# vision-agh/apse_uav

Measured on AMD Instinct MI355X. Metric: 4K UAV frames/sec (whole node), higher is better.
Workload: dtype f32

## Files before the change

### apse_uav_amd/_lib.py

```python
import ctypes as C
import os

import numpy as np

_HERE = os.path.dirname(os.path.abspath(__file__))
_TREE_LIB = os.path.join(_HERE, "libapse_hip.so")
LIB_PATH = os.environ.get("APSE_HIP_LIB") or _TREE_LIB
TOOL_ENTRIES = ("apse_winograd_pack_filter", "apse_winograd_conv2d", "apse_lane_stats", "apse_rpn_select", "apse_box_inference",
                "apse_c4_rpn_select", "apse_rpn_select_train", "apse_rpn_train_proposals_workspace_bytes", "apse_rpn_train_proposals",
                "apse_set_rpn_head", "apse_preprocess_frames_yuv", "apse_yuv_to_bgr", "apse_yuv_matrix_host", "apse_resize_normalize_yuv")

APSE_OK = 0


class ApseError(RuntimeError):
    pass


class Config(C.Structure):
    _fields_ = [
        ("struct_size", C.c_int), ("device", C.c_int), ("max_batch", C.c_int),
        ("frame_h", C.c_int), ("frame_w", C.c_int), ("image_h", C.c_int), ("image_w", C.c_int),
        ("blocks", C.c_int * 4), ("num_classes", C.c_int),
        ("score_thresh", C.c_float), ("box_nms", C.c_float), ("rpn_nms", C.c_float), ("mask_thresh", C.c_float),
        ("rpn_pre_topk", C.c_int), ("rpn_post_topk", C.c_int), ("dets_per_image", C.c_int),
        ("pixel_mean", C.c_float * 3), ("assoc_roi", C.c_int), ("embed_dim", C.c_int), ("assoc_scale", C.c_float),
        ("compute_dtype", C.c_int), ("storage16", C.c_int),
    ]


class ConfigArch(Config):
# ... 48 lines not shown
    "apse_set_detections": ([vp, vp, vp, vp, vp, i, vp], i),
    "apse_mask_tail": ([vp, i, vp], i),
    "apse_embed": ([vp, i, vp], i),
    "apse_forward": ([vp, i, vp], i),
    "apse_results_describe": ([vp, C.POINTER(ResultsLayout)], i),
    "apse_read_results": ([vp, vp, sz, vp], i),
    "apse_read_results_begin": ([vp, vp, sz, vp], i),
    "apse_read_results_end": ([vp, vp], i),
    "apse_lane_stats": ([vp, C.POINTER(C.c_longlong * 4)], i),
    "apse_copy_mask_window": ([vp, i, i, i, i, i, vp, vp], i),
    "apse_copy_mask_windows": ([vp, i, vp, vp, vp, vp, vp], i),
    "apse_host_copy": ([vp, vp, sz, i], i),
    "apse_feature_shape": ([vp, C.c_char_p, C.POINTER(C.c_int * 3)], i),
    "apse_export_feature": ([vp, C.c_char_p, vp, i, vp], i),
    "apse_debug_tensor": ([vp, C.c_char_p, vp, sz, C.POINTER(sz), vp], i),
    "apse_flops": ([vp, i, C.c_double, C.c_double], C.c_double),
    "apse_profile": ([vp, i], i),
    "apse_profile_read": ([vp, C.POINTER(C.c_double * 42), i], i),
    "apse_conv_packed_elems": ([C.POINTER(ConvDesc)], sz),
    "apse_conv_pack_weight": ([C.POINTER(ConvDesc), vp, i, vp, vp], i),
    "apse_conv2d": ([C.POINTER(ConvDesc), vp, vp, vp, vp, vp, vp, sz, vp], i),
    "apse_winograd_pack_filter": ([vp, i, i, vp], i),
    "apse_winograd_conv2d": ([C.POINTER(ConvDesc), vp, vp, vp, vp, vp], i),
    "apse_maxpool3x3s2": ([vp, vp, i, i, i, i, vp], i),
    "apse_maxpool3x3s2_typed": ([vp, vp, i, i, i, i, i, vp], i),
    "apse_roi_align": ([C.POINTER(vp), C.POINTER(i), C.POINTER(i), vp, i, i, i, vp, vp], i),
    "apse_roi_align_typed": ([C.POINTER(vp), C.POINTER(i), C.POINTER(i), vp, i, i, i, i, vp, vp], i),
    "apse_roi_pool": ([vp, i, i, vp, vp, i, i, f, vp, vp], i),
    "apse_roi_features": ([vp, i, vp, vp, i, i, vp, vp], i),
    "apse_nms_rank": ([vp, vp, vp, i, i, i, i, f, i, vp, vp, vp, vp, vp], i),
    "apse_rpn_select": ([C.POINTER(vp), C.POINTER(i), C.POINTER(i), i, i, i, i, i, i, f, i, vp, vp, vp, vp, vp, vp, vp, vp, vp], i),
    "apse_box_inference": ([vp, i, i, vp, vp, i, i, i, i, f, f, i, i] + [vp] * 16, i),
    "apse_c4_rpn_select": ([vp, i, i, i, i, i, i, i, f, vp, vp, vp, vp, vp, vp, vp, vp], i),
    "apse_mask_centroid_dense": ([vp, i, i, C.POINTER(C.c_int * 3), vp], i),
    "apse_mask_closest_dense": ([vp, i, i, f, f, C.POINTER(C.c_int * 2), vp], i),
    "apse_l2_normalize": ([vp, vp, i, i, vp], i),
    "apse_sqdist": ([vp, vp, i, i, i, vp, vp], i),
    "apse_undistort_gamma": ([vp, vp, i, i, i, C.POINTER(C.c_double), C.POINTER(C.c_double), i, vp, i, i, vp], i),
    "apse_lab_tables_host": ([vp, vp, C.c_size_t], C.c_size_t),
    "apse_replay_create": ([i, i, f, i], vp),
    "apse_replay_destroy": ([vp], None),
    "apse_replay_step": ([vp, i, i, vp, vp, vp, C.c_char_p, i, vp], i),
    "apse_replay_packed": ([vp, vp, C.c_longlong, i, i, i, vp, C.c_longlong], C.c_longlong),
    "apse_replay_max_id": ([vp], i),
    "apse_replay_next_id": ([vp], i),
    "apse_render_workspace_bytes": ([i, i, i], sz),
# ... 116 lines not shown
```

### apse_uav_amd/csrc/apse_common.h

```cpp
#pragma once
#include <hip/hip_runtime.h>
#include <stdint.h>

#define APSE_OK 0
#define APSE_E_INVALID (-1)
#define APSE_E_HIP (-2)
#define APSE_E_NOMEM (-3)
#define APSE_E_STATE (-4)
#define APSE_E_MISSING (-5)
#define APSE_MAX_FRAME_W 49152
#define APSE_MAX_FRAME_H 32768
#define APSE_MAX_CLASSES 80
#define APSE_LDS_BYTES 163840

int apse_fail_global(int code, const char* msg);

typedef __attribute__((ext_vector_type(16))) float f32x16;
typedef __attribute__((ext_vector_type(4))) float f32x4;

struct ConvParams {
    const float* x;
    const float* w;
    const uint16_t* w16;
    const float* bias;
// ... 2 lines not shown
    float* ws;
    int* tile_cnt;
    const int* m_count;
    int m_per_item;
    int m_hint;
    int B, H, W, cin_log2;
    int OH, OW, Cout;
    int KH, KW, stride, pad;
    int KWCp;
    int M;
    int relu;
    int res_mode;
    int out_mode;
    int y_ld, y_coff;
    int cdec;
    int splitk;
    int steps_total;
    const void* next_w;
    unsigned next_w_bytes;
    int prec;
    int x_st, res_st, y_st;
    int no_stream;
    const float* wu;
};

int apse_launch_conv(const ConvParams& p, int cfg, hipStream_t s, hipEvent_t ev0 = nullptr, hipEvent_t ev1 = nullptr);
int apse_conv_pick_cfg(int M, int Cout, int steps, int* splitk);
#define APSE_CFG_STREAM 9
#define APSE_CFG_BNECK 10
#define APSE_CFG_GLDS 11
#define APSE_CFG_STEMPOOL 12
#define APSE_CFG_SKINNY 13
#define APSE_NCFG 14
bool apse_conv1x1_stream_ok(const ConvParams& p);
int apse_launch_conv1x1_stream(const ConvParams& p, hipStream_t s, hipEvent_t ev0 = nullptr, hipEvent_t ev1 = nullptr);
bool apse_conv_glds16_ok(const ConvParams& p);
bool apse_conv_glds16_small(const ConvParams& p);
bool apse_conv_skinny_ok(const ConvParams& p);
int apse_launch_conv_skinny(const ConvParams& p, hipStream_t s, hipEvent_t ev0 = nullptr, hipEvent_t ev1 = nullptr);
int apse_launch_conv_glds16(const ConvParams& p, hipStream_t s, hipEvent_t ev0 = nullptr, hipEvent_t ev1 = nullptr);
int apse_conv_effective_cfg(const ConvParams& p, int cfg);
bool apse_conv_winograd_ok(const ConvParams& p, int max_items);
int apse_conv_winograd_blocks(const ConvParams& p);
int apse_launch_conv_winograd(const ConvParams& p, hipStream_t s, hipEvent_t ev0 = nullptr, hipEvent_t ev1 = nullptr);
typedef __bf16 bf16x8 __attribute__((ext_vector_type(8)));

#ifdef __HIPCC__
typedef _Float16 f16x4_t __attribute__((ext_vector_type(4)));
typedef __bf16 bf16x4_t __attribute__((ext_vector_type(4)));
__device__ __forceinline__ int apse_xcd_remap(int wg, int nwg) {
    const int q = nwg >> 3, r = nwg & 7, xcd = wg & 7, idx = wg >> 3;
    return (xcd < r ? xcd * (q + 1) : r * (q + 1) + (xcd - r) * q) + idx;
}
__device__ __forceinline__ f32x4 apse_ld4(const void* base, size_t idx, int st) {
    if (st == 0) return *reinterpret_cast<const f32x4*>(reinterpret_cast<const float*>(base) + idx);
    f32x4 r;
    if (st == 1) {
        const uint2 raw = *reinterpret_cast<const uint2*>(reinterpret_cast<const uint16_t*>(base) + idx);
        r[0] = __uint_as_float(raw.x << 16); r[1] = __uint_as_float(raw.x & 0xffff0000u);
        r[2] = __uint_as_float(raw.y << 16); r[3] = __uint_as_float(raw.y & 0xffff0000u);
    } else {
        const f16x4_t h = *reinterpret_cast<const f16x4_t*>(reinterpret_cast<const uint16_t*>(base) + idx);
        r[0] = (float)h[0]; r[1] = (float)h[1]; r[2] = (float)h[2]; r[3] = (float)h[3];
    }
    return r;
}
// ... 88 lines not shown
```

### apse_uav_amd/csrc/conv_igemm.hip

```cpp
#include "apse_common.h"
#include <type_traits>

typedef _Float16 f16x8 __attribute__((ext_vector_type(8)));
__device__ __forceinline__ f32x16 apse_mfma16(bf16x8 a, bf16x8 b, f32x16 c) { return __builtin_amdgcn_mfma_f32_32x32x16_bf16(a, b, c, 0, 0, 0); }
__device__ __forceinline__ f32x16 apse_mfma16(f16x8 a, f16x8 b, f32x16 c) { return __builtin_amdgcn_mfma_f32_32x32x16_f16(a, b, c, 0, 0, 0); }

template <int WM, int WN, int TM, int TN, int KS, int XT, int WK, int PR = 0>
__global__ __launch_bounds__(64 * WM * WN * WK) void conv_igemm_f32(const ConvParams p) {
    static_assert(PR == 0 || XT == 0, "16-bit operands use the descriptor path only");
    constexpr bool DESC = XT != 1;
    constexpr int EPS = PR ? 64 : 32;
    constexpr int ESH = PR ? 1 : 2;
    constexpr int EPSLOT = 16 >> ESH;
    constexpr int NT = 64 * WM * WN * WK;
    constexpr int BM = WM * TM * 32;
    constexpr int BN = WN * TN * 32;
    constexpr int SR = NT / 8;
    constexpr int AP = BM / SR;
    constexpr int BP = BN / SR;
    static_assert(AP >= 1 && BP >= 1 && KS % WK == 0 && (DESC || WK == 1), "unsupported shape");
    constexpr int LDC = BN + 4;
    constexpr bool DP = DESC && (TM * TN <= 2 || (PR != 0 && WM * WN == 8 && APSE_DP16));
    constexpr int NSET = DP ? 2 : 1;
    constexpr int STORE_AT = 4 * KS - 2;
// ... 584 lines not shown
        if (p.out_mode == 0) {
            if (p.res_mode == 1) {
                val += ld1((size_t)m * p.Cout + n);
            } else if (p.res_mode == 2) {
                const int b = m / ohw;
                const int rem = m - b * ohw;
                const int oy = rem / p.OW, ox = rem - oy * p.OW;
                const int hw2 = (p.OH >> 1) * (p.OW >> 1);
                val += ld1(((size_t)b * hw2 + (oy >> 1) * (p.OW >> 1) + (ox >> 1)) * p.Cout + n);
            }
            dst = (size_t)m * p.y_ld + p.y_coff + n;
        } else {
            const int b = m / ohw;
            const int rem = m - b * ohw;
            const int oy = rem / p.OW, ox = rem - oy * p.OW;
            const int dy = g >> 1, dx = g & 1;
            dst = (((size_t)b * 2 * p.OH + 2 * oy + dy) * (2 * p.OW) + 2 * ox + dx) * p.cdec + co;
        }
        if (p.relu) val = apse_relu(val);
        apse_st1(p.y, dst, val, p.y_st);
    }
}

template <int WM, int WN, int TM, int TN, int KS, int XT, int WK = 1, int PR = 0>
static int launch_cfg_x(const ConvParams& p, hipStream_t s, hipEvent_t ev0, hipEvent_t ev1) {
    constexpr int BM = WM * TM * 32, BN = WN * TN * 32;
    const int tiles = ((p.M + BM - 1) / BM) * ((p.Cout + BN - 1) / BN);
    const size_t lds_stage = (size_t)2 * KS * (BM + BN) * 32 * sizeof(float), lds_c = (size_t)WK * BM * (BN + 4) * sizeof(float) + 16;
    const size_t lds = lds_stage > lds_c ? lds_stage : lds_c;
    static bool attr_done = false;
    if (!attr_done) {
        hipFuncSetAttribute(reinterpret_cast<const void*>(&conv_igemm_f32<WM, WN, TM, TN, KS, XT, WK, PR>),
                            hipFuncAttributeMaxDynamicSharedMemorySize, (int)lds);
        attr_done = true;
    }
    int grid_x = tiles;
    if (p.m_count) {
        int want = 1024;
        if (p.m_hint > 0) {
            want = 2 * ((p.m_hint + BM - 1) / BM) * ((p.Cout + BN - 1) / BN);
            if (want < 64) want = 64;
            if (want > 1024) want = 1024;
        }
        if (grid_x > want) grid_x = want;
    }
    if (ev0) hipEventRecord(ev0, s);
// ... 138 lines not shown
```

### apse_uav_amd/csrc/conv_winograd.hip

```cpp
#include "apse_common.h"

namespace {
constexpr int WTR = 16, WTC = 4;
constexpr int WT = WTR * WTC;
constexpr int WN = 64;
constexpr int KC = 8;
constexpr int NTHR = 512;
constexpr int G_U = 1, G_ROWS = 2, G_V = 3;
constexpr int SLICE_F = 16 * WT * KC;
constexpr size_t WINO_LDS = (size_t)2 * 2 * SLICE_F * sizeof(float);
static_assert(WN == WT, "V and U slices share one size");
static_assert((size_t)16 * WT * 32 * sizeof(float) <= WINO_LDS, "epilogue chunk must fit the staging LDS");
}

__global__ __launch_bounds__(NTHR) void conv_winograd_f32(const ConvParams p) {
    extern __shared__ __attribute__((aligned(16))) char smem[];
    float* Vs = reinterpret_cast<float*>(smem);
    float* Us = Vs + 2 * SLICE_F;
    float* Cs = reinterpret_cast<float*>(smem);

    const int tid = threadIdx.x;
    const int lane = tid & 63, wave = __builtin_amdgcn_readfirstlane(tid >> 6);
    const int fr = lane & 31, fh = lane >> 5;

    const int tiles_y = (p.OH + 2 * WTR - 1) / (2 * WTR), tiles_x = (p.OW + 2 * WTC - 1) / (2 * WTC);
    const int nblk = p.Cout / WN;
    const int nwg = p.B * tiles_y * tiles_x * nblk;
    const int bid = apse_xcd_remap(blockIdx.x, nwg);
    const int nb = bid % nblk;
    int rest = bid / nblk;
    const int bx = rest % tiles_x; rest /= tiles_x;
    const int by = rest % tiles_y;
    const int b = rest / tiles_y;
    const int oy0 = by * 2 * WTR, ox0 = bx * 2 * WTC, n0 = nb * WN;
    const int C = 1 << p.cin_log2;
    const int nsteps = C / KC;

    const int cg = tid & 1, t = (tid >> 1) & (WT - 1), ti = wave >> 1;
    const int ra = ti == 0 ? 0 : (ti == 2 ? 2 : 1);
    const int rb = ti == 0 ? 2 : (ti == 1 ? 2 : (ti == 2 ? 1 : 3));
    const float sgn = ti == 1 ? 1.f : -1.f;
    const int iy_a = oy0 + 2 * (t / WTC) - 1 + ra, iy_b = oy0 + 2 * (t / WTC) - 1 + rb;
    const int ix0 = ox0 + 2 * (t % WTC) - 1;
    const __amdgpu_buffer_rsrc_t xrsrc =
        __builtin_amdgcn_make_buffer_rsrc(const_cast<float*>(p.x), 0, (int)((((unsigned)(p.B * p.H * p.W)) << p.cin_log2) * 4u), 0x00020000);
    const __amdgpu_buffer_rsrc_t xnone = __builtin_amdgcn_make_buffer_rsrc(const_cast<float*>(p.x), 0, 0, 0x00020000);
    unsigned xoff[2][4];
#pragma unroll
    for (int r = 0; r < 2; ++r) {
        const int iy = r ? iy_b : iy_a;
#pragma unroll
        for (int c = 0; c < 4; ++c) {
            const int ix = ix0 + c;
            const bool in = (unsigned)iy < (unsigned)p.H && (unsigned)ix < (unsigned)p.W;
            xoff[r][c] = in ? ((((unsigned)((b * p.H + iy) * p.W + ix)) << p.cin_log2) + (unsigned)(cg * 4)) * 4u : 0x80000000u;
        }
    }
    const __amdgpu_buffer_rsrc_t ursrc =
        __builtin_amdgcn_make_buffer_rsrc(const_cast<float*>(p.wu), 0, (int)((((unsigned)(16 * p.Cout)) << p.cin_log2) * 4u), 0x00020000);
    const unsigned ustep = (unsigned)(16 * p.Cout * KC * 4);
    unsigned uoff[4], ulds[4];
#pragma unroll
    for (int k = 0; k < 4; ++k) {
        const int q = tid + NTHR * k;
        const int xi = q >> 7, co = (q >> 1) & 63, h = q & 1;
        uoff[k] = (unsigned)(((xi * p.Cout + n0 + co) * KC + h * 4) * 4);
        ulds[k] = (unsigned)((xi * WN + co) * KC + ((h ^ ((co >> 3) & 1)) * 4));
    }
    const int vlds = (4 * ti * WT + t) * KC + (cg ^ ((t >> 3) & 1)) * 4;

    f32x4 xr[2][4], ur[4];
    auto fetch_u = [&](int s) {
        const unsigned kb = (unsigned)s * ustep;
#pragma unroll
        for (int k = 0; k < 4; ++k) ur[k] = __builtin_bit_cast(f32x4, __builtin_amdgcn_raw_buffer_load_b128(ursrc, (int)(uoff[k] + kb), 0, 0));
    };
    auto fetch_x = [&](int s) {
        const unsigned kb = (unsigned)(s * KC * 4);
        const __amdgpu_buffer_rsrc_t rs = s < nsteps ? xrsrc : xnone;
#pragma unroll
        for (int r = 0; r < 2; ++r)
#pragma unroll
            for (int c = 0; c < 4; ++c)
                xr[r][c] = __builtin_bit_cast(f32x4, __builtin_amdgcn_raw_buffer_load_b128(rs, (int)(xoff[r][c] + kb), 0, 0));
    };
    auto write_u = [&](int buf) {
#pragma unroll
        for (int k = 0; k < 4; ++k) *reinterpret_cast<f32x4*>(Us + buf * SLICE_F + ulds[k]) = ur[k];
    };
    auto xform_rows = [&]() {
#pragma unroll
        for (int c = 0; c < 4; ++c)
#pragma unroll
            for (int e = 0; e < 4; ++e) xr[0][c][e] = __builtin_fmaf(xr[1][c][e], sgn, xr[0][c][e]);
    };
    auto write_v = [&](int buf) {
        const f32x4 v[4] = {xr[0][0] - xr[0][2], xr[0][1] + xr[0][2], xr[0][2] - xr[0][1], xr[0][1] - xr[0][3]};
#pragma unroll
        for (int j = 0; j < 4; ++j) *reinterpret_cast<f32x4*>(Vs + buf * SLICE_F + vlds + j * WT * KC) = v[j];
    };

// ... 58 lines not shown
    typedef unsigned u32x4_t __attribute__((ext_vector_type(4)));
#pragma unroll
    for (int j = 0; j < 2; ++j) {
#pragma unroll
        for (int a = 0; a < 2; ++a)
#pragma unroll
            for (int i = 0; i < 2; ++i)
#pragma unroll
                for (int v = 0; v < 16; ++v) {
                    const int row = 32 * i + (v & 3) + 8 * (v >> 2) + 4 * fh;
                    Cs[((2 * wave + a) * WT + row) * 32 + fr] = acc[a][i][j][v];
                }
        __syncthreads();
        f32x4 m[16];
#pragma unroll
        for (int k = 0; k < 16; ++k) m[k] = *reinterpret_cast<const f32x4*>(Cs + (k * WT + et) * 32 + eg * 4);
        f32x4 s0[4], s1[4];
#pragma unroll
        for (int c = 0; c < 4; ++c) {
            s0[c] = m[c] + m[4 + c] + m[8 + c];
            s1[c] = m[4 + c] - m[8 + c] - m[12 + c];
        }
        const int co = n0 + 32 * j + 4 * eg;
        const f32x4 bias4 = p.bias ? *reinterpret_cast<const f32x4*>(p.bias + co) : f32x4{0.f, 0.f, 0.f, 0.f};
        f32x4 y[2][2] = {{s0[0] + s0[1] + s0[2], s0[1] - s0[2] - s0[3]}, {s1[0] + s1[1] + s1[2], s1[1] - s1[2] - s1[3]}};
#pragma unroll
        for (int dy = 0; dy < 2; ++dy)
#pragma unroll
            for (int dx = 0; dx < 2; ++dx) {
                f32x4 val = y[dy][dx] + bias4;
                if (p.relu) {
#pragma unroll
                    for (int k = 0; k < 4; ++k) val[k] = apse_relu(val[k]);
                }
                if (oy + dy < p.OH && ox + dx < p.OW)
                    APSE_NT_STORE(val, reinterpret_cast<f32x4*>(p.y + ((size_t)(b * p.OH + oy + dy) * p.OW + ox + dx) * p.y_ld + p.y_coff + co));
            }
        __syncthreads();
    }
}

bool apse_conv_winograd_ok(const ConvParams& p, int max_items) {
    return p.prec == 0 && p.x_st == 0 && p.y_st == 0 && p.KH == 3 && p.KW == 3 && p.stride == 1 && p.pad == 1 && p.out_mode == 0 &&
           p.res_mode == 0 && p.splitk == 1 && p.Cout % WN == 0 && p.cin_log2 >= 3 && p.OH == p.H && p.OW == p.W &&
           (p.y_ld & 3) == 0 && (p.y_coff & 3) == 0 && ((((size_t)max_items * p.H * p.W) << p.cin_log2) * 4 < 0x7fff0000ull);
}

int apse_conv_winograd_blocks(const ConvParams& p) {
    return ((p.OH + 2 * WTR - 1) / (2 * WTR)) * ((p.OW + 2 * WTC - 1) / (2 * WTC)) * (p.Cout / WN);
}

int apse_launch_conv_winograd(const ConvParams& p, hipStream_t s, hipEvent_t ev0, hipEvent_t ev1) {
    if (!p.wu || !apse_conv_winograd_ok(p, p.B) || p.m_count) return APSE_E_INVALID;
    static bool attr_done = false;
    if (!attr_done) {
        hipFuncSetAttribute(reinterpret_cast<const void*>(&conv_winograd_f32), hipFuncAttributeMaxDynamicSharedMemorySize, (int)WINO_LDS);
        attr_done = true;
    }
    const int tiles_y = (p.OH + 2 * WTR - 1) / (2 * WTR), tiles_x = (p.OW + 2 * WTC - 1) / (2 * WTC);
    const int grid = p.B * tiles_y * tiles_x * (p.Cout / WN);
    if (ev0) hipEventRecord(ev0, s);
    hipLaunchKernelGGL(conv_winograd_f32, dim3(grid), dim3(NTHR), WINO_LDS, s, p);
    if (ev1) hipEventRecord(ev1, s);
    return hipGetLastError() == hipSuccess ? APSE_OK : APSE_E_HIP;
}
```

### apse_uav_amd/csrc/ops.hip

```cpp
#include "detector_ctx.h"

#include <math.h>
#include <string.h>

#include <map>
#include <mutex>
#include <vector>

namespace {
struct DevBuf {
    void* p = nullptr;
    ~DevBuf() { if (p) hipFree(p); }
    bool alloc(size_t bytes, bool zero = false) {
        if (hipMalloc(&p, bytes ? bytes : 16) != hipSuccess) { p = nullptr; return false; }
        if (zero) hipMemset(p, 0, bytes ? bytes : 16);
        return true;
    }
    template <typename T> T* as() const { return reinterpret_cast<T*>(p); }
};
}

extern "C" {

size_t apse_conv_packed_elems(const apse_conv_desc* d) {
// ... 61 lines not shown
}

int apse_winograd_pack_filter(const float* w, int Cout, int Cin, float* packed) {
    if (!w || !packed || Cout < 1 || Cin < 8 || pow2_at_least(Cin) != Cin) return APSE_E_INVALID;
    const std::vector<float> u = winograd_filters(w, Cout, Cin, Cin);
    memcpy(packed, u.data(), u.size() * sizeof(float));
    return APSE_OK;
}

int apse_winograd_conv2d(const apse_conv_desc* d, const float* x, const float* wu, const float* bias, float* y, void* stream) {
    if (!d || !x || !wu || !y || d->B < 1 || d->H < 1 || d->W < 1 || d->Cin < 8 || pow2_at_least(d->Cin) != d->Cin) return APSE_E_INVALID;
    ConvParams p;
    memset(&p, 0, sizeof p);
    p.x = x; p.wu = wu; p.bias = bias; p.y = y;
    p.B = d->B; p.H = d->H; p.W = d->W; p.cin_log2 = apse_ilog2(d->Cin);
    p.KH = d->KH; p.KW = d->KW; p.stride = d->stride; p.pad = d->pad;
    p.OH = d->H; p.OW = d->W; p.Cout = d->Cout; p.relu = d->relu;
    p.M = p.B * p.OH * p.OW; p.m_per_item = p.OH * p.OW;
    p.y_ld = d->Cout; p.splitk = 1;
    p.res_mode = d->res_mode; p.prec = d->prec; p.x_st = d->x_st; p.y_st = d->y_st;
    return apse_launch_conv_winograd(p, (hipStream_t)stream);
}

int apse_maxpool3x3s2(const float* x, float* y, int B, int H, int W, int C, void* stream) {
    return apse_k_maxpool3x3s2(x, y, B, H, W, C, 0, (hipStream_t)stream);
}

int apse_maxpool3x3s2_typed(const void* x, void* y, int B, int H, int W, int C, int storage, void* stream) {
    if (!x || !y || B < 1 || H < 1 || W < 1 || C < 4 || (C & 3) || storage < 0 || storage > 2) return APSE_E_INVALID;
    return apse_k_maxpool3x3s2(x, y, B, H, W, C, storage, (hipStream_t)stream);
}

static int roi_align_stateless(const void* const* feats, const int* hs, const int* ws, const float* rois, int n, int per_img,
                               int out_size, int st, void* out, void* stream) {
    if (!feats || !hs || !ws || !rois || !out || n < 0 || out_size < 1 || st < 0 || st > 2) return APSE_E_INVALID;
    FpnMaps F;
    static const float sc[4] = {0.25f, 0.125f, 0.0625f, 0.03125f};
    for (int l = 0; l < 4; ++l) { F.p[l] = feats[l]; F.H[l] = hs[l]; F.W[l] = ws[l]; F.scale[l] = sc[l]; }
    F.st = st;
    static int* total_dev = nullptr;
    if (!total_dev) hipMalloc(reinterpret_cast<void**>(&total_dev), sizeof(int));
    hipMemcpyAsync(total_dev, &n, sizeof(int), hipMemcpyHostToDevice, (hipStream_t)stream);
    hipStreamSynchronize((hipStream_t)stream);
    std::vector<int> img(n);
    for (int i = 0; i < n; ++i) img[i] = per_img > 0 ? i / per_img : 0;
    int* img_dev = nullptr;
// ... 343 lines not shown
```

### apse_uav_amd/csrc/plan.hip

```cpp
#include "detector_ctx.h"

#include <math.h>
#include <stdio.h>
#include <string.h>

#define APSE_WINO_MIN_BLOCKS 128
#define APSE_EXPECTED_DETS 8

void pack_oihw(const float* w, int Cout, int Cin, int KH, int KW, int cin_p, const float* scale, float* out, int KWCp) {
    for (int o = 0; o < Cout; ++o) {
        const float sc = scale ? scale[o] : 1.0f;
        for (int r = 0; r < KH; ++r)
            for (int s = 0; s < KW; ++s)
                for (int ci = 0; ci < Cin; ++ci)
                    out[((size_t)o * KH + r) * KWCp + s * cin_p + ci] = w[(((size_t)o * Cin + ci) * KH + r) * KW + s] * sc;
    }
}

static const HostW* getw(apse_ctx* c, const std::string& n) {
    auto it = c->hw.find(n);
    return it == c->hw.end() ? nullptr : &it->second;
}

static Tens make_t(apse_ctx* c, const std::string& name, int items, int H, int W, int C, int st = 0) {
    Tens t;
    t.H = H; t.W = W; t.C = C; t.st = st;
    const size_t elems = (size_t)items * H * W * C;
    t.p = dalloc<float>(c, st ? (elems + 1) / 2 : elems);
    c->t[name] = t;
// ... 11 lines not shown
    const Tens* res = nullptr; int res_mode = 0;
    int y_ld = 0;
    int count_kind = 0;
    float* out_ptr = nullptr;
    const Tens* out_view = nullptr;
};

static uint16_t round16(float v, int dtype) {
    if (dtype == 2) {
        const _Float16 hval = (_Float16)v;
        uint16_t r;
        memcpy(&r, &hval, 2);
        return r;
    }
    uint32_t b;
    memcpy(&b, &v, 4);
    if ((b & 0x7fffffffu) > 0x7f800000u) return (uint16_t)((b >> 16) | 0x40);
    return (uint16_t)((b + 0x7fffu + ((b >> 16) & 1u)) >> 16);
}
static int storage_type(const apse_ctx* c) { return (c->cfg.compute_dtype >= 1 && c->cfg.storage16) ? c->cfg.compute_dtype : 0; }

static bool winograd_layer(const std::string& n) {
    return n == "backbone.fpn_output2" || n == "backbone.fpn_output3" || n == "rpn_t2" || n == "rpn_t3";
}
std::vector<float> winograd_filters(const float* oihw, int Cout, int Cin, int cin_p) {
    static const double G[4][3] = {{1, 0, 0}, {0.5, 0.5, 0.5}, {0.5, -0.5, 0.5}, {0, 0, 1}};
    std::vector<float> u((size_t)16 * Cout * cin_p, 0.f);
    for (int o = 0; o < Cout; ++o)
        for (int ci = 0; ci < Cin; ++ci) {
            const float* g = oihw + ((size_t)o * Cin + ci) * 9;
            double t[4][3];
            for (int i = 0; i < 4; ++i)
                for (int s = 0; s < 3; ++s) t[i][s] = G[i][0] * g[s] + G[i][1] * g[3 + s] + G[i][2] * g[6 + s];
            for (int i = 0; i < 4; ++i)
                for (int j = 0; j < 4; ++j) {
                    const double v = t[i][0] * G[j][0] + t[i][1] * G[j][1] + t[i][2] * G[j][2];
                    u[(((size_t)(ci / 8) * 16 + 4 * i + j) * Cout + o) * 8 + (ci & 7)] = (float)v;
                }
        }
    return u;
}

static int add_conv(apse_ctx* c, std::vector<Step>& plan, const ConvSpec& sp, const Tens& in, Tens* out) {
    const std::string& out_name = sp.out_name.empty() ? sp.name : sp.out_name;
    std::vector<float> rows;
    std::vector<float> bias;
// ... 118 lines not shown
    Tens o;
    if (sp.out_view) { o = *sp.out_view; o.H = oh; o.W = ow; o.C = out_c; c->t[out_name] = o; }
    else if (sp.out_ptr) { o.p = sp.out_ptr; o.H = oh; o.W = ow; o.C = out_c; }
    else o = make_t(c, out_name, c->cfg.max_batch * sp.items, oh, ow, out_c, out_st);
    p.y_st = o.st;
    if (!o.p) return fail(c, APSE_E_NOMEM, "activation alloc failed at " + sp.name);
    p.y = o.p; p.y_ld = out_c; p.y_coff = 0;
    cs.flops_per_item = sp.s2d ? 2.0 * p.OH * p.OW * (double)Cout * 7 * 7 * 3
                               : 2.0 * p.OH * p.OW * (double)Cout * KH * KW * Cin;
    const int Mfull = c->cfg.max_batch * sp.items * p.OH * p.OW;
    int sk = 1;
    cs.cfg = apse_conv_pick_cfg(Mfull, Cout, p.steps_total, &sk);
    if (sp.count_kind == 2) {
        const int kd = c->cfg.dets_per_image < APSE_EXPECTED_DETS ? c->cfg.dets_per_image : APSE_EXPECTED_DETS;
        const int rows = kd * c->cfg.max_batch * p.OH * p.OW;
        sk = 1;
        cs.cfg = apse_conv_pick_cfg(rows < Mfull ? rows : Mfull, Cout, p.steps_total, &sk);
    }
    p.splitk = sk;
    if (sk > 1) {
        const size_t need = (size_t)sk * Mfull * Cout;
        if (need > c->ws_floats) c->ws_floats = need;
    }
    if (c->f32_winograd && winograd_layer(sp.name) && sp.count_kind == 0 && apse_conv_winograd_ok(p, c->cfg.max_batch * sp.items) &&
        apse_conv_winograd_blocks(p) >= APSE_WINO_MIN_BLOCKS) {
        p.wu = dupload(c, winograd_filters(rows.data(), Cout, Cin, cin_p));
        if (!p.wu) return fail(c, APSE_E_NOMEM, "weight upload failed at " + sp.name);
    }
    if (out) *out = o;
    plan.push_back(st);
    return APSE_OK;
}

static void layout_results(apse_ctx* c) {
    apse_results_layout& L = c->lay;
    memset(&L, 0, sizeof(L));
    const int B = c->cfg.max_batch, kd = c->cfg.dets_per_image, n = B * kd, E = c->cfg.embed_dim;
    L.n_max = n; L.dets_per_image = kd; L.embed_dim = E; L.max_batch = B;
    size_t o = 0;
    auto take = [&](size_t bytes) { size_t r = o; o += (bytes + 15) / 16 * 16; return r; };
    L.total = take(4);
    L.offset = take(4 * (B + 1));
    L.prop_count = take(4 * B);
    L.img = take(4 * n); L.cls = take(4 * n); L.roi = take(4 * n); L.score = take(4 * n);
    L.box_resized = take(16 * n); L.box = take(16 * n); L.valid = take(4 * n); L.rect = take(16 * n);
    L.mass = take(4 * n); L.centroid = take(8 * n);
    L.closest = take((size_t)8 * n * kd);
    L.embedding = take((size_t)4 * n * E);
    L.bytes = o;
}
// ... 480 lines not shown
```

### apse_uav_amd/winograd.py

```python
import numpy as np

BT = np.array([[1, 0, -1, 0], [0, 1, 1, 0], [0, -1, 1, 0], [0, 1, 0, -1]], dtype=np.float64)
G = np.array([[1, 0, 0], [0.5, 0.5, 0.5], [0.5, -0.5, 0.5], [0, 0, 1]], dtype=np.float64)
AT = np.array([[1, 1, 1, 0], [0, 1, -1, -1]], dtype=np.float64)


def filter_transform(w):
    w = np.asarray(w, dtype=np.float64)
    u = np.einsum("ir,ocrs,js->ijoc", G, w, G)
    return u.reshape(16, w.shape[0], w.shape[1]).astype(np.float32)


def _input_transform(d):
    d0, d1, d2, d3 = d[..., 0, :, :], d[..., 1, :, :], d[..., 2, :, :], d[..., 3, :, :]
    rows = [d0 - d2, d1 + d2, d2 - d1, d1 - d3]
    v = []
    for x in rows:
        x0, x1, x2, x3 = x[..., 0, :], x[..., 1, :], x[..., 2, :], x[..., 3, :]
        v += [x0 - x2, x1 + x2, x2 - x1, x1 - x3]
    return np.stack(v, axis=-2)


def _output_transform(m):
    q = [m[..., k, :] for k in range(16)]
    s0 = [q[0 + j] + q[4 + j] + q[8 + j] for j in range(4)]
    s1 = [q[4 + j] - q[8 + j] - q[12 + j] for j in range(4)]
    y00 = s0[0] + s0[1] + s0[2]
    y01 = s0[1] - s0[2] - s0[3]
    y10 = s1[0] + s1[1] + s1[2]
    y11 = s1[1] - s1[2] - s1[3]
    return np.stack([np.stack([y00, y01], -2), np.stack([y10, y11], -2)], -3)


def emulate(x_hwc, w_oihw, bias, relu):
    x = np.asarray(x_hwc, dtype=np.float32)
    H, W, C = x.shape
    th, tw = (H + 1) // 2, (W + 1) // 2
    xp = np.zeros((2 * th + 2, 2 * tw + 2, C), np.float32)
    xp[1:H + 1, 1:W + 1] = x
    iy = (2 * np.arange(th))[:, None] + np.arange(4)[None, :]
    ix = (2 * np.arange(tw))[:, None] + np.arange(4)[None, :]
    d = xp[iy[:, None, :, None], ix[None, :, None, :]]
    v = _input_transform(d)
    u = filter_transform(w_oihw)
    m = np.zeros((th, tw, 16, u.shape[1]), np.float32)
    uc = np.ascontiguousarray(u.transpose(2, 0, 1))
    rows = max(1, (1 << 18) // (tw * 16 * u.shape[1]))
    for r0 in range(0, th, rows):
        vr, mr = v[r0:r0 + rows], m[r0:r0 + rows]
        for c in range(C):
            mr += vr[..., c:c + 1] * uc[c]
    y = _output_transform(m) + np.asarray(bias, np.float32)
    if relu:
        y = np.maximum(y, 0)
    y = y.transpose(0, 2, 1, 3, 4).reshape(2 * th, 2 * tw, -1)
    return y[:H, :W]
```

### include/apse_hip.h

```cpp
#ifndef APSE_HIP_H
#define APSE_HIP_H
#include <stddef.h>
#include <stdint.h>
#ifdef __cplusplus
extern "C" {
#endif

#define APSE_OK 0
#define APSE_E_INVALID (-1)
#define APSE_E_HIP (-2)
#define APSE_E_NOMEM (-3)
#define APSE_E_STATE (-4)
#define APSE_E_MISSING (-5)

typedef struct apse_ctx apse_ctx;

#define APSE_MAX_CLASSES 80
#define APSE_C4_MAX_PRE_TOPK 6000
#define APSE_C4_MAX_BATCH 2
#define APSE_MAX_FRAME_W 49152
#define APSE_MAX_FRAME_H 32768
typedef struct apse_config {
    int struct_size;
    int device;
// ... 82 lines not shown
double apse_flops(apse_ctx* ctx, int batch, double proposals, double detections);

int apse_profile(apse_ctx* ctx, int enable);
int apse_profile_read(apse_ctx* ctx, double* out42, int reset);

typedef struct apse_conv_desc {
    int B, H, W, Cin;
    int Cout, KH, KW, stride, pad;
    int relu;
    int res_mode;
    int cfg;
    int splitk;
    int prec;
    int fuse_reduce;
    int x_st, res_st, y_st;
} apse_conv_desc;
size_t apse_conv_packed_elems(const apse_conv_desc* d);
int apse_conv_pack_weight(const apse_conv_desc* d, const float* w_oihw, int cin_real, const float* scale, float* packed);
int apse_conv2d(const apse_conv_desc* d, const float* x_dev, const float* w_packed_dev, const float* bias_dev,
                const float* res_dev, float* y_dev, float* ws_dev, size_t ws_bytes, void* stream);
int apse_winograd_pack_filter(const float* w_oihw, int Cout, int Cin, float* packed);
int apse_winograd_conv2d(const apse_conv_desc* d, const float* x_dev, const float* wu_dev, const float* bias_dev, float* y_dev,
                         void* stream);
int apse_maxpool3x3s2(const float* x_dev, float* y_dev, int B, int H, int W, int C, void* stream);
int apse_maxpool3x3s2_typed(const void* x_dev, void* y_dev, int B, int H, int W, int C, int storage, void* stream);
int apse_roi_align(const float* const* feats_dev, const int* hs, const int* ws, const float* rois_dev, int n, int per_img,
                   int out_size, float* out_dev, void* stream);
int apse_roi_align_typed(const void* const* feats_dev, const int* hs, const int* ws, const float* rois_dev, int n, int per_img,
                         int out_size, int storage, void* out_dev, void* stream);
int apse_roi_pool(const float* feat_dev, int H, int W, const float* rois_dev, const int* roi_img_dev, int n, int out_size,
                  float scale, float* out_dev, void* stream);
int apse_nms_rank(const float* boxes_dev, const float* scores_dev, const int* valid_dev, int n, int cat_div, int cat_mod,
                  int ncat, float thr, int topk, float* out_boxes_dev, float* out_scores_dev, int* out_index_dev,
                  int* out_count_dev, void* stream);
int apse_rpn_select(const float* const* heads_dev, const int* H, const int* W, int head_ld, int B, int image_h, int image_w,
                    int pre_topk, int post_topk, float nms_thr, int level_mask, unsigned long long* keys_dev, float* dec_boxes_dev,
                    float* dec_scores_dev, int* dec_valid_dev, float* props_dev, float* prop_scores_dev, int* prop_entry_dev,
                    int* prop_count_dev, void* stream);
int apse_box_inference(const float* pred_dev, int ld, int K, const float* props_dev, const int* prop_cnt_dev, int P, int B,
                       int image_h, int image_w, float score_thresh, float nms_thr, int dets_per_image, int wide,
                       float* probs_dev, float* cand_boxes_dev, float* cand_scores_dev, int* cand_valid_dev, float* det_boxes_dev,
                       float* det_scores_dev, int* det_entry_dev, int* det_cnt_dev, float* pk_boxes_dev, float* pk_scores_dev,
                       int* pk_cls_dev, int* pk_img_dev, int* pk_roi_dev, int* pk_total_dev, int* pk_offset_dev, void* stream);
int apse_c4_rpn_select(const float* head_dev, int H, int W, int B, int image_h, int image_w, int pre, int post, float nms_thr,
                       float* dec_boxes_dev, float* dec_scores_dev, int* dec_valid_dev, float* props_dev, float* prop_scores_dev,
                       int* prop_entry_dev, int* prop_count_dev, void* stream);
// ... 224 lines not shown
```

Before: 203.6.

## Extend Winograd conv to trunk 3x3 layers with split-K and alternate tile geometry

```diff
diff --git a/apse_uav_amd/_lib.py b/apse_uav_amd/_lib.py
--- a/apse_uav_amd/_lib.py
+++ b/apse_uav_amd/_lib.py
@@ -6,7 +6,7 @@
 _HERE = os.path.dirname(os.path.abspath(__file__))
 _TREE_LIB = os.path.join(_HERE, "libapse_hip.so")
 LIB_PATH = os.environ.get("APSE_HIP_LIB") or _TREE_LIB
-TOOL_ENTRIES = ("apse_winograd_pack_filter", "apse_winograd_conv2d", "apse_lane_stats", "apse_rpn_select", "apse_box_inference",
+TOOL_ENTRIES = ("apse_winograd_pack_filter", "apse_winograd_conv2d", "apse_winograd_conv2d_split", "apse_lane_stats", "apse_rpn_select", "apse_box_inference",
                 "apse_c4_rpn_select", "apse_rpn_select_train", "apse_rpn_train_proposals_workspace_bytes", "apse_rpn_train_proposals",
                 "apse_set_rpn_head", "apse_preprocess_frames_yuv", "apse_yuv_to_bgr", "apse_yuv_matrix_host", "apse_resize_normalize_yuv")
 
@@ -101,6 +101,7 @@
     "apse_conv2d": ([C.POINTER(ConvDesc), vp, vp, vp, vp, vp, vp, sz, vp], i),
     "apse_winograd_pack_filter": ([vp, i, i, vp], i),
     "apse_winograd_conv2d": ([C.POINTER(ConvDesc), vp, vp, vp, vp, vp], i),
+    "apse_winograd_conv2d_split": ([C.POINTER(ConvDesc), vp, vp, vp, vp, vp, C.c_size_t, i, vp], i),
     "apse_maxpool3x3s2": ([vp, vp, i, i, i, i, vp], i),
     "apse_maxpool3x3s2_typed": ([vp, vp, i, i, i, i, i, vp], i),
     "apse_roi_align": ([C.POINTER(vp), C.POINTER(i), C.POINTER(i), vp, i, i, i, vp, vp], i),
diff --git a/apse_uav_amd/csrc/apse_common.h b/apse_uav_amd/csrc/apse_common.h
--- a/apse_uav_amd/csrc/apse_common.h
+++ b/apse_uav_amd/csrc/apse_common.h
@@ -48,6 +48,7 @@
     int x_st, res_st, y_st;
     int no_stream;
     const float* wu;
+    int wino_geom;
 };
 
 int apse_launch_conv(const ConvParams& p, int cfg, hipStream_t s, hipEvent_t ev0 = nullptr, hipEvent_t ev1 = nullptr);
@@ -68,6 +69,7 @@
 int apse_conv_effective_cfg(const ConvParams& p, int cfg);
 bool apse_conv_winograd_ok(const ConvParams& p, int max_items);
 int apse_conv_winograd_blocks(const ConvParams& p);
+void apse_launch_splitk_reduce4(const ConvParams& p, hipStream_t s);
 int apse_launch_conv_winograd(const ConvParams& p, hipStream_t s, hipEvent_t ev0 = nullptr, hipEvent_t ev1 = nullptr);
 typedef __bf16 bf16x8 __attribute__((ext_vector_type(8)));
 
diff --git a/apse_uav_amd/csrc/conv_igemm.hip b/apse_uav_amd/csrc/conv_igemm.hip
--- a/apse_uav_amd/csrc/conv_igemm.hip
+++ b/apse_uav_amd/csrc/conv_igemm.hip
@@ -630,6 +630,12 @@
     }
 }
 
+void apse_launch_splitk_reduce4(const ConvParams& p, hipStream_t s) {
+    int blocks = (int)(((size_t)p.M * p.Cout / 4 + 255) / 256);
+    if (blocks > 4096) blocks = 4096;
+    hipLaunchKernelGGL(conv_splitk_reduce4, dim3(blocks), dim3(256), 0, s, p);
+}
+
 template <int WM, int WN, int TM, int TN, int KS, int XT, int WK = 1, int PR = 0>
 static int launch_cfg_x(const ConvParams& p, hipStream_t s, hipEvent_t ev0, hipEvent_t ev1) {
     constexpr int BM = WM * TM * 32, BN = WN * TN * 32;
diff --git a/apse_uav_amd/csrc/conv_winograd.hip b/apse_uav_amd/csrc/conv_winograd.hip
--- a/apse_uav_amd/csrc/conv_winograd.hip
+++ b/apse_uav_amd/csrc/conv_winograd.hip
@@ -1,8 +1,7 @@
 #include "apse_common.h"
 
 namespace {
-constexpr int WTR = 16, WTC = 4;
-constexpr int WT = WTR * WTC;
+constexpr int WT = 64;
 constexpr int WN = 64;
 constexpr int KC = 8;
 constexpr int NTHR = 512;
@@ -13,7 +12,9 @@
 static_assert((size_t)16 * WT * 32 * sizeof(float) <= WINO_LDS, "epilogue chunk must fit the staging LDS");
 }
 
+template <int WTR, int WTC, bool SPLIT>
 __global__ __launch_bounds__(NTHR) void conv_winograd_f32(const ConvParams p) {
+    static_assert(WTR * WTC == WT, "64 tiles per block");
     extern __shared__ __attribute__((aligned(16))) char smem[];
     float* Vs = reinterpret_cast<float*>(smem);
     float* Us = Vs + 2 * SLICE_F;
@@ -34,7 +35,13 @@
     const int b = rest / tiles_y;
     const int oy0 = by * 2 * WTR, ox0 = bx * 2 * WTC, n0 = nb * WN;
     const int C = 1 << p.cin_log2;
-    const int nsteps = C / KC;
+    int s_begin = 0, s_end = C / KC;
+    if constexpr (SPLIT) {
+        const int z = blockIdx.y, share = s_end / p.splitk, extra = s_end % p.splitk;
+        s_begin = z * share + (z < extra ? z : extra);
+        s_end = s_begin + share + (z < extra ? 1 : 0);
+    }
+    const int nsteps = s_end - s_begin;
 
     const int cg = tid & 1, t = (tid >> 1) & (WT - 1), ti = wave >> 1;
     const int ra = ti == 0 ? 0 : (ti == 2 ? 2 : 1);
@@ -56,9 +63,9 @@
             xoff[r][c] = in ? ((((unsigned)((b * p.H + iy) * p.W + ix)) << p.cin_log2) + (unsigned)(cg * 4)) * 4u : 0x80000000u;
         }
     }
-    const __amdgpu_buffer_rsrc_t ursrc =
-        __builtin_amdgcn_make_buffer_rsrc(const_cast<float*>(p.wu), 0, (int)((((unsigned)(16 * p.Cout)) << p.cin_log2) * 4u), 0x00020000);
     const unsigned ustep = (unsigned)(16 * p.Cout * KC * 4);
+    const __amdgpu_buffer_rsrc_t ursrc = __builtin_amdgcn_make_buffer_rsrc(
+        const_cast<float*>(p.wu), 0, SPLIT ? (int)((unsigned)s_end * ustep) : (int)((((unsigned)(16 * p.Cout)) << p.cin_log2) * 4u), 0x00020000);
     unsigned uoff[4], ulds[4];
 #pragma unroll
     for (int k = 0; k < 4; ++k) {
@@ -71,12 +78,12 @@
 
     f32x4 xr[2][4], ur[4];
     auto fetch_u = [&](int s) {
-        const unsigned kb = (unsigned)s * ustep;
+        const unsigned kb = (unsigned)(s_begin + s) * ustep;
 #pragma unroll
         for (int k = 0; k < 4; ++k) ur[k] = __builtin_bit_cast(f32x4, __builtin_amdgcn_raw_buffer_load_b128(ursrc, (int)(uoff[k] + kb), 0, 0));
     };
     auto fetch_x = [&](int s) {
-        const unsigned kb = (unsigned)(s * KC * 4);
+        const unsigned kb = (unsigned)((s_begin + s) * KC * 4);
         const __amdgpu_buffer_rsrc_t rs = s < nsteps ? xrsrc : xnone;
 #pragma unroll
         for (int r = 0; r < 2; ++r)
@@ -181,6 +188,19 @@
             s1[c] = m[4 + c] - m[8 + c] - m[12 + c];
         }
         const int co = n0 + 32 * j + 4 * eg;
+        if constexpr (SPLIT) {
+            float* slab = p.ws + (size_t)blockIdx.y * p.M * p.Cout;
+#pragma unroll
+            for (int dy = 0; dy < 2; ++dy)
+#pragma unroll
+                for (int dx = 0; dx < 2; ++dx) {
+                    const f32x4 val = dy ? (dx ? s1[1] - s1[2] - s1[3] : s1[0] + s1[1] + s1[2]) : (dx ? s0[1] - s0[2] - s0[3] : s0[0] + s0[1] + s0[2]);
+                    if (oy + dy < p.OH && ox + dx < p.OW)
+                        *reinterpret_cast<f32x4*>(slab + ((size_t)(b * p.OH + oy + dy) * p.OW + ox + dx) * p.Cout + co) = val;
+                }
+            __syncthreads();
+            continue;
+        }
         const f32x4 bias4 = p.bias ? *reinterpret_cast<const f32x4*>(p.bias + co) : f32x4{0.f, 0.f, 0.f, 0.f};
         f32x4 y[2][2] = {{s0[0] + s0[1] + s0[2], s0[1] - s0[2] - s0[3]}, {s1[0] + s1[1] + s1[2], s1[1] - s1[2] - s1[3]}};
 #pragma unroll
@@ -201,25 +221,36 @@
 
 bool apse_conv_winograd_ok(const ConvParams& p, int max_items) {
     return p.prec == 0 && p.x_st == 0 && p.y_st == 0 && p.KH == 3 && p.KW == 3 && p.stride == 1 && p.pad == 1 && p.out_mode == 0 &&
-           p.res_mode == 0 && p.splitk == 1 && p.Cout % WN == 0 && p.cin_log2 >= 3 && p.OH == p.H && p.OW == p.W &&
+           p.res_mode == 0 && p.Cout % WN == 0 && p.cin_log2 >= 3 && p.splitk >= 1 && p.splitk <= (1 << p.cin_log2) / KC &&
+           (p.wino_geom == 0 || p.wino_geom == 1) && p.OH == p.H && p.OW == p.W &&
            (p.y_ld & 3) == 0 && (p.y_coff & 3) == 0 && ((((size_t)max_items * p.H * p.W) << p.cin_log2) * 4 < 0x7fff0000ull);
 }
 
 int apse_conv_winograd_blocks(const ConvParams& p) {
-    return ((p.OH + 2 * WTR - 1) / (2 * WTR)) * ((p.OW + 2 * WTC - 1) / (2 * WTC)) * (p.Cout / WN);
+    const int wtr = p.wino_geom ? 8 : 16, wtc = p.wino_geom ? 8 : 4;
+    return ((p.OH + 2 * wtr - 1) / (2 * wtr)) * ((p.OW + 2 * wtc - 1) / (2 * wtc)) * (p.Cout / WN);
+}
+
+template <int WTR, int WTC, bool SPLIT>
+static void launch_wino(const ConvParams& p, int grid, hipStream_t s) {
+    static bool attr_done = false;
+    if (!attr_done) {
+        hipFuncSetAttribute(reinterpret_cast<const void*>(&conv_winograd_f32<WTR, WTC, SPLIT>), hipFuncAttributeMaxDynamicSharedMemorySize,
+                            (int)WINO_LDS);
+        attr_done = true;
+    }
+    hipLaunchKernelGGL((conv_winograd_f32<WTR, WTC, SPLIT>), dim3(grid, SPLIT ? p.splitk : 1), dim3(NTHR), WINO_LDS, s, p);
 }
 
 int apse_launch_conv_winograd(const ConvParams& p, hipStream_t s, hipEvent_t ev0, hipEvent_t ev1) {
     if (!p.wu || !apse_conv_winograd_ok(p, p.B) || p.m_count) return APSE_E_INVALID;
-    static bool attr_done = false;
-    if (!attr_done) {
-        hipFuncSetAttribute(reinterpret_cast<const void*>(&conv_winograd_f32), hipFuncAttributeMaxDynamicSharedMemorySize, (int)WINO_LDS);
-        attr_done = true;
-    }
-    const int tiles_y = (p.OH + 2 * WTR - 1) / (2 * WTR), tiles_x = (p.OW + 2 * WTC - 1) / (2 * WTC);
-    const int grid = p.B * tiles_y * tiles_x * (p.Cout / WN);
+    const bool split = p.splitk > 1;
+    if (split && (!p.ws || p.tile_cnt || p.M != p.B * p.OH * p.OW || (size_t)p.M * p.Cout >= 0x7fffffffull)) return APSE_E_INVALID;
+    const int grid = p.B * apse_conv_winograd_blocks(p);
     if (ev0) hipEventRecord(ev0, s);
-    hipLaunchKernelGGL(conv_winograd_f32, dim3(grid), dim3(NTHR), WINO_LDS, s, p);
+    if (p.wino_geom == 0) { if (split) launch_wino<16, 4, true>(p, grid, s); else launch_wino<16, 4, false>(p, grid, s); }
+    else { if (split) launch_wino<8, 8, true>(p, grid, s); else launch_wino<8, 8, false>(p, grid, s); }
     if (ev1) hipEventRecord(ev1, s);
+    if (split) apse_launch_splitk_reduce4(p, s);
     return hipGetLastError() == hipSuccess ? APSE_OK : APSE_E_HIP;
 }
diff --git a/apse_uav_amd/csrc/ops.hip b/apse_uav_amd/csrc/ops.hip
--- a/apse_uav_amd/csrc/ops.hip
+++ b/apse_uav_amd/csrc/ops.hip
@@ -107,6 +107,23 @@
     return apse_launch_conv_winograd(p, (hipStream_t)stream);
 }
 
+int apse_winograd_conv2d_split(const apse_conv_desc* d, const float* x, const float* wu, const float* bias, float* y, float* ws,
+                               size_t ws_bytes, int geometry, void* stream) {
+    if (!d || !x || !wu || !y || d->B < 1 || d->H < 1 || d->W < 1 || d->Cin < 8 || pow2_at_least(d->Cin) != d->Cin) return APSE_E_INVALID;
+    if (d->splitk < 1 || d->splitk > d->Cin / 8 || (geometry != 0 && geometry != 1)) return APSE_E_INVALID;
+    ConvParams p;
+    memset(&p, 0, sizeof p);
+    p.x = x; p.wu = wu; p.bias = bias; p.y = y; p.ws = ws;
+    p.B = d->B; p.H = d->H; p.W = d->W; p.cin_log2 = apse_ilog2(d->Cin);
+    p.KH = d->KH; p.KW = d->KW; p.stride = d->stride; p.pad = d->pad;
+    p.OH = d->H; p.OW = d->W; p.Cout = d->Cout; p.relu = d->relu;
+    p.M = p.B * p.OH * p.OW; p.m_per_item = p.OH * p.OW;
+    p.y_ld = d->Cout; p.splitk = d->splitk; p.wino_geom = geometry;
+    p.res_mode = d->res_mode; p.prec = d->prec; p.x_st = d->x_st; p.y_st = d->y_st;
+    if (p.splitk > 1 && (!ws || (size_t)p.splitk * p.M * p.Cout * sizeof(float) > ws_bytes)) return APSE_E_INVALID;
+    return apse_launch_conv_winograd(p, (hipStream_t)stream);
+}
+
 int apse_maxpool3x3s2(const float* x, float* y, int B, int H, int W, int C, void* stream) {
     return apse_k_maxpool3x3s2(x, y, B, H, W, C, 0, (hipStream_t)stream);
 }
diff --git a/apse_uav_amd/csrc/plan.hip b/apse_uav_amd/csrc/plan.hip
--- a/apse_uav_amd/csrc/plan.hip
+++ b/apse_uav_amd/csrc/plan.hip
@@ -5,6 +5,8 @@
 #include <string.h>
 
 #define APSE_WINO_MIN_BLOCKS 128
+#define APSE_WINO_TRUNK_MIN_TILES 1000
+#define APSE_WINO_GRID 256
 #define APSE_EXPECTED_DETS 8
 
 void pack_oihw(const float* w, int Cout, int Cin, int KH, int KW, int cin_p, const float* scale, float* out, int KWCp) {
@@ -62,6 +64,27 @@
 
 static bool winograd_layer(const std::string& n) {
     return n == "backbone.fpn_output2" || n == "backbone.fpn_output3" || n == "rpn_t2" || n == "rpn_t3";
+}
+static bool winograd_trunk_layer(const std::string& n) {
+    static const std::string trunk = "backbone.bottom_up.res", c2 = ".conv2";
+    if (n == "backbone.fpn_output4" || n == "rpn_t4") return true;
+    return n.size() > trunk.size() + c2.size() && n.compare(0, trunk.size(), trunk) == 0 && n[trunk.size()] != '4' &&
+           n.compare(n.size() - c2.size(), c2.size(), c2) == 0;
+}
+static void winograd_trunk_shape(ConvParams& p) {
+    const int slices = (1 << p.cin_log2) / 8;
+    int best = -1;
+    for (int g = 0; g < 2; ++g) {
+        ConvParams q = p;
+        q.wino_geom = g;
+        const int nb = apse_conv_winograd_blocks(q);
+        int sk = nb >= APSE_WINO_GRID ? 1 : APSE_WINO_GRID / nb;
+        if (sk > slices) sk = slices;
+        const int grid = nb * sk, over = grid > APSE_WINO_GRID;
+        const int score = over ? -grid : grid;
+        const bool better = best == -1 || score > best || (score == best && sk > 1);
+        if (better) { best = score; p.wino_geom = g; p.splitk = sk; }
+    }
 }
 std::vector<float> winograd_filters(const float* oihw, int Cout, int Cin, int cin_p) {
     static const double G[4][3] = {{1, 0, 0}, {0.5, 0.5, 0.5}, {0.5, -0.5, 0.5}, {0, 0, 1}};
@@ -226,10 +249,26 @@
         const size_t need = (size_t)sk * Mfull * Cout;
         if (need > c->ws_floats) c->ws_floats = need;
     }
-    if (c->f32_winograd && winograd_layer(sp.name) && sp.count_kind == 0 && apse_conv_winograd_ok(p, c->cfg.max_batch * sp.items) &&
-        apse_conv_winograd_blocks(p) >= APSE_WINO_MIN_BLOCKS) {
-        p.wu = dupload(c, winograd_filters(rows.data(), Cout, Cin, cin_p));
-        if (!p.wu) return fail(c, APSE_E_NOMEM, "weight upload failed at " + sp.name);
+    if (c->f32_winograd && sp.count_kind == 0) {
+        ConvParams q = p;
+        bool take = false;
+        if (winograd_layer(sp.name)) {
+            take = sk == 1 && apse_conv_winograd_ok(q, c->cfg.max_batch * sp.items) && apse_conv_winograd_blocks(q) >= APSE_WINO_MIN_BLOCKS;
+        } else if (!c->c4 && winograd_trunk_layer(sp.name) &&
+                   ((c->PH / 16 + 1) / 2) * ((c->PW / 16 + 1) / 2) >= APSE_WINO_TRUNK_MIN_TILES) {
+            q.splitk = 1;
+            if (apse_conv_winograd_ok(q, c->cfg.max_batch * sp.items)) {
+                winograd_trunk_shape(q);
+                take = apse_conv_winograd_ok(q, c->cfg.max_batch * sp.items);
+            }
+        }
+        if (take) {
+            p = q;
+            p.wu = dupload(c, winograd_filters(rows.data(), Cout, Cin, cin_p));
+            if (!p.wu) return fail(c, APSE_E_NOMEM, "weight upload failed at " + sp.name);
+            const size_t need = (size_t)p.splitk * Mfull * Cout;
+            if (p.splitk > 1 && need > c->ws_floats) c->ws_floats = need;
+        }
     }
     if (out) *out = o;
     plan.push_back(st);
diff --git a/apse_uav_amd/winograd.py b/apse_uav_amd/winograd.py
--- a/apse_uav_amd/winograd.py
+++ b/apse_uav_amd/winograd.py
@@ -32,7 +32,19 @@
     return np.stack([np.stack([y00, y01], -2), np.stack([y10, y11], -2)], -3)
 
 
-def emulate(x_hwc, w_oihw, bias, relu):
+def split_ranges(cin, split):
+    slices = cin // 8
+    assert cin % 8 == 0 and 1 <= split <= slices
+    share, extra = divmod(slices, split)
+    out, s = [], 0
+    for z in range(split):
+        n = share + (1 if z < extra else 0)
+        out.append((8 * s, 8 * (s + n)))
+        s += n
+    return out
+
+
+def emulate(x_hwc, w_oihw, bias, relu, split=1):
     x = np.asarray(x_hwc, dtype=np.float32)
     H, W, C = x.shape
     th, tw = (H + 1) // 2, (W + 1) // 2
@@ -46,11 +58,22 @@
     m = np.zeros((th, tw, 16, u.shape[1]), np.float32)
     uc = np.ascontiguousarray(u.transpose(2, 0, 1))
     rows = max(1, (1 << 18) // (tw * 16 * u.shape[1]))
-    for r0 in range(0, th, rows):
-        vr, mr = v[r0:r0 + rows], m[r0:r0 + rows]
-        for c in range(C):
-            mr += vr[..., c:c + 1] * uc[c]
-    y = _output_transform(m) + np.asarray(bias, np.float32)
+    if split == 1:
+        for r0 in range(0, th, rows):
+            vr, mr = v[r0:r0 + rows], m[r0:r0 + rows]
+            for c in range(C):
+                mr += vr[..., c:c + 1] * uc[c]
+        y = _output_transform(m) + np.asarray(bias, np.float32)
+    else:
+        y = np.zeros((th, tw, 2, 2, u.shape[1]), np.float32)
+        for c0, c1 in split_ranges(C, split):
+            m[...] = 0
+            for r0 in range(0, th, rows):
+                vr, mr = v[r0:r0 + rows], m[r0:r0 + rows]
+                for c in range(c0, c1):
+                    mr += vr[..., c:c + 1] * uc[c]
+            y += _output_transform(m)
+        y = y + np.asarray(bias, np.float32)
     if relu:
         y = np.maximum(y, 0)
     y = y.transpose(0, 2, 1, 3, 4).reshape(2 * th, 2 * tw, -1)
diff --git a/include/apse_hip.h b/include/apse_hip.h
--- a/include/apse_hip.h
+++ b/include/apse_hip.h
@@ -128,6 +128,8 @@
 int apse_winograd_pack_filter(const float* w_oihw, int Cout, int Cin, float* packed);
 int apse_winograd_conv2d(const apse_conv_desc* d, const float* x_dev, const float* wu_dev, const float* bias_dev, float* y_dev,
                          void* stream);
+int apse_winograd_conv2d_split(const apse_conv_desc* d, const float* x_dev, const float* wu_dev, const float* bias_dev, float* y_dev,
+                               float* ws_dev, size_t ws_bytes, int geometry, void* stream);
 int apse_maxpool3x3s2(const float* x_dev, float* y_dev, int B, int H, int W, int C, void* stream);
 int apse_maxpool3x3s2_typed(const void* x_dev, void* y_dev, int B, int H, int W, int C, int storage, void* stream);
 int apse_roi_align(const float* const* feats_dev, const int* hs, const int* ws, const float* rois_dev, int n, int per_img,
```

After: 207.1, median of 6. +1.7%, better.
